# uingei/hevc

Hardware: AMD Instinct MI355X
Metric: encoded 1080p30 frames/sec/GPU; PSNR-Y parity vs libx265 at matched bitrate (higher is better)
Workload: dtype u8; 1 GPU; 1920x1080@30 SDR 8-bit Main, crf 19 capped by VBV maxrate 2940 kbps / bufsize 3528 kbit (the reference's libx265 operating point), 300-frame synthetic 'motion' clip per GPU, keyint 90 (4 closed GOPs of equal length), IPPP, full-search +-15, one clip per GPU, input resident in HBM

## Files before the change

### hevc_amd/csrc/kernels/common.h

```cpp
#pragma once
#include <stdint.h>

#if defined(__HIPCC__)
#include <hip/hip_runtime.h>
#define DEV __device__ __forceinline__
#define HD __host__ __device__
#define HDI __host__ __device__ inline
#define DEVCONST __device__ const
#define MIHEVC_GPU 1
#else
#define DEV inline
#define HD
#define HDI inline
#define DEVCONST static const
#define MIHEVC_GPU 0
#endif

#include "../../../include/mihevc.h"

namespace mihevc {

constexpr int CTU = 32;
constexpr int CTU_LOG2 = 5;
constexpr int PAD_Y = 80;
// ... 75 lines not shown
                         5, 5, 6, 6, 7, 8, 9, 10, 11, 13, 14, 16, 18, 20, 22, 24};
    for (int i = 0; i < 54; i++) t.tc[i] = (uint8_t)tcv[i];
    const int qs[6] = {26214, 23302, 20560, 18396, 16384, 14564}, ls[6] = {40, 45, 51, 57, 64, 72};
    for (int i = 0; i < 6; i++) { t.quant_scale[i] = (int16_t)qs[i]; t.level_scale[i] = (uint8_t)ls[i]; }
    const int cq[14] = {29, 30, 31, 32, 33, 33, 34, 34, 35, 35, 36, 36, 37, 37};
    for (int i = 0; i < 14; i++) t.chroma_qp[i] = (int8_t)cq[i];
    for (int ty = 0; ty < 4; ty++)
        for (int tx = 0; tx < 4; tx++) t.zorder[ty * 4 + tx] = (uint8_t)(((ty >> 1) * 2 + (tx >> 1)) * 4 + (ty & 1) * 2 + (tx & 1));
    return t;
}
DEVCONST Tables g_tab = make_tables();

DEV int iabs(int v) { return v < 0 ? -v : v; }
DEV int imin(int a, int b) { return a < b ? a : b; }
DEV int imax(int a, int b) { return a > b ? a : b; }
DEV int clip3(int lo, int hi, int v) { return v < lo ? lo : v > hi ? hi : v; }
DEV int ilog2u(unsigned v) { return 31 - __builtin_clz(v | 1); }
DEV int mvd_bits(int d)
{
    int a = iabs(d);
    return a == 0 ? 1 : a == 1 ? 3 : 3 + 2 * ilog2u((unsigned)a);
}
DEV int chroma_qp_of(int qp)
{
    int q = clip3(-12, 57, qp);
    return q < 30 ? q : q > 43 ? q - 6 : g_tab.chroma_qp[q - 30];
}
DEV int zaddr(int x, int y, int ctus_w)
{
    int bx = (x & 31) >> 2, by = (y & 31) >> 2, z = 0;
    for (int i = 0; i < 3; i++) z |= ((bx >> i) & 1) << (2 * i) | ((by >> i) & 1) << (2 * i + 1);
    return (((y >> CTU_LOG2) * ctus_w + (x >> CTU_LOG2)) << 6) | z;
}
DEV void node_geom(int node, int &x, int &y, int &log2n)
{
    if (node == 0) { x = 0; y = 0; log2n = 5; }
    else if (node < 5) { int q = node - 1; x = (q & 1) * 16; y = (q >> 1) * 16; log2n = 4; }
    else { int q = (node - 5) >> 2, s = (node - 5) & 3; x = (q & 1) * 16 + (s & 1) * 8; y = (q >> 1) * 16 + (s >> 1) * 8; log2n = 3; }
}
DEV int node_of_tile(int level, int tx, int ty)
{
    if (level == 0) return 0;
    int q = (ty >> 1) * 2 + (tx >> 1);
    return level == 1 ? 1 + q : 5 + q * 4 + (ty & 1) * 2 + (tx & 1);
}

DEV uint32_t sad_packed_u8(uint32_t a, uint32_t b, uint32_t acc)
{
#if MIHEVC_GPU
    return __builtin_amdgcn_sad_u8(a, b, acc);
#else
    for (int i = 0; i < 4; i++) acc += (uint32_t)iabs((int)((a >> (8 * i)) & 255) - (int)((b >> (8 * i)) & 255));
    return acc;
#endif
}
DEV uint32_t sad_packed_u16(uint32_t a, uint32_t b, uint32_t acc)
{
#if MIHEVC_GPU
    return __builtin_amdgcn_sad_u16(a, b, acc);
#else
    for (int i = 0; i < 2; i++) acc += (uint32_t)iabs((int)((a >> (16 * i)) & 65535) - (int)((b >> (16 * i)) & 65535));
    return acc;
#endif
}
DEV uint32_t load_u32(const void *p)
{
    uint32_t v;
    __builtin_memcpy(&v, p, 4);
    return v;
}
DEV uint32_t sad_row8(const uint8_t *a, const uint8_t *b, uint32_t acc)
{
    acc = sad_packed_u8(load_u32(a), load_u32(b), acc);
    return sad_packed_u8(load_u32(a + 4), load_u32(b + 4), acc);
}
DEV uint32_t sad_row8(const uint16_t *a, const uint16_t *b, uint32_t acc)
{
    for (int i = 0; i < 8; i += 2) acc = sad_packed_u16(load_u32(a + i), load_u32(b + i), acc);
    return acc;
}

DEV uint32_t pk_add16(uint32_t a, uint32_t b)
{
#if MIHEVC_GPU
    typedef short v2s __attribute__((ext_vector_type(2)));
    return __builtin_bit_cast(uint32_t, (v2s)(__builtin_bit_cast(v2s, a) + __builtin_bit_cast(v2s, b)));
#else
    return ((a + b) & 0xffffu) | (((a >> 16) + (b >> 16)) << 16);
#endif
}
DEV uint32_t pk_sub16(uint32_t a, uint32_t b)
{
#if MIHEVC_GPU
    typedef short v2s __attribute__((ext_vector_type(2)));
    return __builtin_bit_cast(uint32_t, (v2s)(__builtin_bit_cast(v2s, a) - __builtin_bit_cast(v2s, b)));
#else
    return ((a - b) & 0xffffu) | (((a >> 16) - (b >> 16)) << 16);
#endif
}
DEV uint32_t pk_max_i16(uint32_t a, uint32_t b)
{
#if MIHEVC_GPU
    uint32_t r;
    asm("v_pk_max_i16 %0, %1, %2" : "=v"(r) : "v"(a), "v"(b));
    return r;
#else
    const int al = (int16_t)(a & 0xffffu), ah = (int16_t)(a >> 16), bl = (int16_t)(b & 0xffffu), bh = (int16_t)(b >> 16);
    return (uint32_t)((al > bl ? al : bl) & 0xffff) | ((uint32_t)((ah > bh ? ah : bh) & 0xffff) << 16);
#endif
}

DEV uint32_t perm_bytes(uint32_t a, uint32_t b, uint32_t sel)
{
#if MIHEVC_GPU
    return __builtin_amdgcn_perm(a, b, sel);
#else
    const uint64_t ab = ((uint64_t)a << 32) | b;
    uint32_t r = 0;
    for (int i = 0; i < 4; i++) r |= (uint32_t)((ab >> (8 * ((sel >> (8 * i)) & 7))) & 255u) << (8 * i);
    return r;
#endif
}
DEV void transpose_bytes4(const uint32_t (&r)[4], uint32_t (&c)[4])
{
    const uint32_t t0 = perm_bytes(r[1], r[0], 0x05010400u), t1 = perm_bytes(r[1], r[0], 0x07030602u);
    const uint32_t t2 = perm_bytes(r[3], r[2], 0x05010400u), t3 = perm_bytes(r[3], r[2], 0x07030602u);
    c[0] = perm_bytes(t2, t0, 0x05040100u); c[1] = perm_bytes(t2, t0, 0x07060302u);
    c[2] = perm_bytes(t3, t1, 0x05040100u); c[3] = perm_bytes(t3, t1, 0x07060302u);
}

DEV bool wave_all(bool p)
{
#if MIHEVC_GPU
    return __all(p) != 0;
#else
    return p;
#endif
}

DEV uint64_t qsad_u8(uint64_t ref8, uint32_t cur, uint64_t acc)
{
#if MIHEVC_GPU
    return __builtin_amdgcn_qsad_pk_u16_u8(ref8, cur, acc);
#else
    uint64_t out = 0;
    for (int j = 0; j < 4; j++) {
        uint32_t w = (uint32_t)(ref8 >> (8 * j)), a = (uint32_t)((acc >> (16 * j)) & 0xffff);
        for (int i = 0; i < 4; i++) a += (uint32_t)iabs((int)((w >> (8 * i)) & 255) - (int)((cur >> (8 * i)) & 255));
        out |= (uint64_t)(a & 0xffff) << (16 * j);
    }
    return out;
#endif
}
DEV uint32_t align_bytes(uint32_t hi, uint32_t lo, int shift_bytes)
{
#if MIHEVC_GPU
    return __builtin_amdgcn_alignbyte(hi, lo, (uint32_t)shift_bytes);
#else
    return (uint32_t)(((((uint64_t)hi) << 32) | lo) >> (8 * shift_bytes));
#endif
}
template <typename T>
DEV void copy_window(T *lds, int ls, const T *plane, int pstride, int ox, int oy, int w, int h, int lo_x, int hi_x, int lo_y, int hi_y, int tid)
{
    constexpr int per = 4 / (int)sizeof(T);
    constexpr int CH = 6;
    const int dpr = w / per, col = tid & 31, rg = tid >> 5;
    for (int d = col; d < dpr; d += 32) {
        const int x = clip3(lo_x, hi_x - (per - 1), ox + d * per);
        for (int r0 = rg; r0 < h; r0 += CH * (NT / 32)) {
            uint32_t v[CH];
#pragma unroll
            for (int k = 0; k < CH; k++) {
                const int r = r0 + k * (NT / 32);
                if (r < h) v[k] = load_u32(plane + (ptrdiff_t)clip3(lo_y, hi_y, oy + r) * pstride + x);
            }
#pragma unroll
            for (int k = 0; k < CH; k++) {
                const int r = r0 + k * (NT / 32);
                if (r < h) __builtin_memcpy(__builtin_assume_aligned(lds + r * ls + d * per, 4), &v[k], 4);
            }
        }
    }
}

template <typename T>
DEV void load_ctu_source(T *dst, const Plane<const T> (&src)[3], int x0, int y0, int w, int h, int tid)
{
    constexpr int per = 4 / (int)sizeof(T);
    if (x0 + CTU <= w && y0 + CTU <= h) {
        constexpr int ND = 1536 / per, IT = (ND + NT - 1) / NT;
        uint32_t v[IT];
#pragma unroll
        for (int k = 0; k < IT; k++) {
            const int d = tid + k * NT;
            if (d < ND) {
                const int i = d * per, pl = i < 1024 ? 0 : 1 + ((i - 1024) >> 8), kk = pl ? (i - 1024) & 255 : i, x = pl ? kk & 15 : kk & 31, y = pl ? kk >> 4 : kk >> 5;
                v[k] = load_u32(src[pl].p + (size_t)((pl ? y0 >> 1 : y0) + y) * src[pl].stride + (pl ? x0 >> 1 : x0) + x);
            }
        }
#pragma unroll
        for (int k = 0; k < IT; k++) {
            const int d = tid + k * NT;
            if (d < ND) __builtin_memcpy(__builtin_assume_aligned(dst + d * per, 4), &v[k], 4);
        }
        return;
    }
    for (int i = tid; i < 1536; i += NT) {
        int pl, x, y;
        if (i < 1024) { pl = 0; x = i & 31; y = i >> 5; } else { int k = i - 1024; pl = 1 + (k >> 8); k &= 255; x = k & 15; y = k >> 4; }
        const int gx = (pl ? x0 >> 1 : x0) + x, gy = (pl ? y0 >> 1 : y0) + y, pw = pl ? w >> 1 : w, ph = pl ? h >> 1 : h;
        dst[i] = (gx < pw && gy < ph) ? src[pl].p[(size_t)gy * src[pl].stride + gx] : (T)0;
    }
}

DEV int wave_uniform(int v)
{
#if MIHEVC_GPU
    v = __builtin_amdgcn_readfirstlane(v);
#endif
    return v;
}
DEV int opaque_zero()
{
    int z = 0;
#if MIHEVC_GPU
    asm volatile("" : "+v"(z));
#endif
    return z;
}
DEV uint32_t load_u32_aligned(const void *p)
{
    uint32_t v;
    __builtin_memcpy(&v, __builtin_assume_aligned(p, 4), 4);
    return v;
}
DEV void store_u32_aligned(void *p, uint32_t v) { __builtin_memcpy(__builtin_assume_aligned(p, 4), &v, 4); }
DEV void store4(uint8_t *p, int v0, int v1, int v2, int v3) { store_u32_aligned(p, (uint32_t)v0 | (uint32_t)v1 << 8 | (uint32_t)v2 << 16 | (uint32_t)v3 << 24); }
DEV void store4(uint16_t *p, int v0, int v1, int v2, int v3)
{
    store_u32_aligned(p, (uint32_t)v0 | (uint32_t)v1 << 16);
    store_u32_aligned(p + 2, (uint32_t)v2 | (uint32_t)v3 << 16);
}
DEV void store4(int16_t *p, int v0, int v1, int v2, int v3)
{
    store_u32_aligned(p, ((uint32_t)v0 & 0xffffu) | (uint32_t)v1 << 16);
    store_u32_aligned(p + 2, ((uint32_t)v2 & 0xffffu) | (uint32_t)v3 << 16);
}
DEV void load_row15(const uint8_t *base, int idx, int (&px)[15])
{
    const int off = idx & 3;
    const uint8_t *p = base + (idx - off);
    uint32_t d[5];
#pragma unroll
    for (int k = 0; k < 5; k++) d[k] = load_u32_aligned(p + 4 * k);
    uint32_t r[4];
#pragma unroll
    for (int k = 0; k < 4; k++) r[k] = align_bytes(d[k + 1], d[k], off);
#pragma unroll
    for (int i = 0; i < 15; i++) px[i] = (int)((r[i >> 2] >> (8 * (i & 3))) & 255);
}
DEV void load_row15(const uint16_t *base, int idx, int (&px)[15])
{
    const int off = idx & 1;
    const uint16_t *p = base + (idx - off);
    uint32_t d[8];
#pragma unroll
    for (int k = 0; k < 8; k++) d[k] = load_u32_aligned(p + 2 * k);
    uint32_t r[8];
#pragma unroll
    for (int k = 0; k < 7; k++) r[k] = align_bytes(d[k + 1], d[k], 2 * off);
    r[7] = align_bytes(0, d[7], 2 * off);
#pragma unroll
    for (int i = 0; i < 15; i++) px[i] = (int)((r[i >> 1] >> (16 * (i & 1))) & 65535);
}

DEV void load_row8(const uint8_t *base, int idx, int (&px)[8])
{
    const int off = idx & 3;
    const uint8_t *p = base + (idx - off);
    const uint32_t d0 = load_u32_aligned(p), d1 = load_u32_aligned(p + 4), d2 = load_u32_aligned(p + 8);
    const uint32_t r0 = align_bytes(d1, d0, off), r1 = align_bytes(d2, d1, off);
#pragma unroll
    for (int i = 0; i < 4; i++) { px[i] = (int)((r0 >> (8 * i)) & 255); px[4 + i] = (int)((r1 >> (8 * i)) & 255); }
}
DEV void load_row8(const uint16_t *base, int idx, int (&px)[8])
{
    const int off = idx & 1;
    const uint16_t *p = base + (idx - off);
    uint32_t d[5];
#pragma unroll
    for (int k = 0; k < 5; k++) d[k] = load_u32_aligned(p + 2 * k);
#pragma unroll
    for (int k = 0; k < 4; k++) {
        const uint32_t r = align_bytes(d[k + 1], d[k], 2 * off);
        px[2 * k] = (int)(r & 65535); px[2 * k + 1] = (int)(r >> 16);
    }
}

DEV int dot4_i8(uint32_t a, uint32_t b, int acc)
{
#if MIHEVC_GPU
    return __builtin_amdgcn_sdot4((int)a, (int)b, acc, false);
#else
    for (int i = 0; i < 4; i++) acc += (int)(int8_t)(a >> (8 * i)) * (int)(int8_t)(b >> (8 * i));
    return acc;
#endif
}
DEV int dot2_i16(uint32_t a, uint32_t b, int acc)
{
#if MIHEVC_GPU
    typedef short v2s __attribute__((ext_vector_type(2)));
    v2s va, vb;
    __builtin_memcpy(&va, &a, 4);
    __builtin_memcpy(&vb, &b, 4);
    return __builtin_amdgcn_sdot2(va, vb, acc, false);
#else
    return acc + (int)(int16_t)(a & 0xffff) * (int)(int16_t)(b & 0xffff) + (int)(int16_t)(a >> 16) * (int)(int16_t)(b >> 16);
#endif
}

DEV uint32_t pack_lo16(int lo, int hi)
{
#if MIHEVC_GPU
    return __builtin_amdgcn_perm((uint32_t)hi, (uint32_t)lo, 0x05040100u);
#else
    return ((uint32_t)lo & 0xffffu) | ((uint32_t)hi << 16);
#endif
}

DEV int hadamard8_satd(int (&m)[8][8])
{
#pragma unroll
    for (int y = 0; y < 8; y++) {
#pragma unroll
        for (int st = 1; st < 8; st <<= 1)
#pragma unroll
            for (int i = 0; i < 8; i++)
                if (!(i & st)) { int p = m[y][i], q = m[y][i + st]; m[y][i] = p + q; m[y][i + st] = p - q; }
    }
    int s = 0;
#pragma unroll
    for (int x = 0; x < 8; x++) {
#pragma unroll
        for (int st = 1; st < 8; st <<= 1)
#pragma unroll
            for (int i = 0; i < 8; i++)
                if (!(i & st)) { int p = m[i][x], q = m[i + st][x]; m[i][x] = p + q; m[i + st][x] = p - q; }
#pragma unroll
        for (int i = 0; i < 8; i++) s += iabs(m[i][x]);
    }
    return (s + 2) >> 2;
}

DEV int hadamard8_ac(int (&m)[8][8])
{
#pragma unroll
    for (int y = 0; y < 8; y++) {
#pragma unroll
        for (int st = 1; st < 8; st <<= 1)
#pragma unroll
            for (int i = 0; i < 8; i++)
                if (!(i & st)) { int p = m[y][i], q = m[y][i + st]; m[y][i] = p + q; m[y][i + st] = p - q; }
    }
    int s = 0;
#pragma unroll
    for (int x = 0; x < 8; x++) {
#pragma unroll
        for (int st = 1; st < 8; st <<= 1)
#pragma unroll
            for (int i = 0; i < 8; i++)
                if (!(i & st)) { int p = m[i][x], q = m[i + st][x]; m[i][x] = p + q; m[i + st][x] = p - q; }
#pragma unroll
        for (int i = 0; i < 8; i++) if (x || i) s += iabs(m[i][x]);
    }
    return (s + 2) >> 2;
}

#if MIHEVC_GPU
#ifdef MIHEVC_PHASE_PROF
__device__ unsigned long long g_phase_prof[8 * 1024 * 3];
#endif
struct GpuExec {
    static DEV int lane_id()
    {
        int t = (int)threadIdx.x;
        asm volatile("" : "+v"(t));
        return t;
    }
// ... 88 lines not shown
```

### hevc_amd/csrc/kernels/inter.h

```cpp
#pragma once
#include "common.h"
#include "residual.h"

namespace mihevc {

template <typename T> struct InterArgs {
    Plane<const T> src[3];
    Plane<const T> ref[3];
    Plane<T> rec[3];
    int w, h, ctus_w;
    CostParams prm;
    const int16_t *centers;
    int32_t *me;
    mihevc_cu_rec *cu;
    int16_t *coef[3];
    unsigned long long *est;
    int sparse_coef;
    IpInfo *ip;
    Plane<const T> ref1[3];
    const int16_t *centers1;
    int32_t *me1;
};
template <typename T> DEV InterArgs<T> list1_view(const InterArgs<T> &a)
{
    InterArgs<T> b = a;
    for (int i = 0; i < 3; i++) b.ref[i] = a.ref1[i];
    b.centers = a.centers1; b.me = a.me1;
    return b;
}

DEVCONST int8_t kOff[9][2] = {{0, 0}, {-1, -1}, {0, -1}, {1, -1}, {-1, 0}, {1, 0}, {-1, 1}, {0, 1}, {1, 1}};
DEVCONST int8_t kRingSlot[8] = {4, 5, 2, 7, 1, 3, 6, 8};

template <typename T> struct PreArgs {
    Plane<const T> src, ref;
    uint8_t *lsrc, *lref;
    int w, h, bit_depth;
    int16_t *centers;
    unsigned *cost;
};
template <typename T> DEV void lowres_sample(const PreArgs<T> &a, int i)
{
    const int lw = a.w >> 2, n = lw * (a.h >> 2), sh = a.bit_depth - 8;
    if (i >= 2 * n) return;
    const Plane<const T> &p = i < n ? a.src : a.ref;
    const int k = i < n ? i : i - n, x = k % lw, y = k / lw;
    int s = 8 << sh;
#pragma unroll
    for (int j = 0; j < 4; j++) {
        const T *row = p.p + (ptrdiff_t)(4 * y + j) * p.stride + 4 * x;
        if (sizeof(T) == 1) {
            s = (int)sad_packed_u8(load_u32(row), 0u, (uint32_t)s);
        } else
            s += (int)row[0] + (int)row[1] + (int)row[2] + (int)row[3];
    }
    s >>= 4 + sh;
    (i < n ? a.lsrc : a.lref)[k] = (uint8_t)(s < 255 ? s : 255);
}
constexpr int PRE_SPAN = 2 * PRE_RANGE + 1;
constexpr int PRE_WIN_W = 40;
constexpr int PRE_WIN_STRIDE = 96;
struct PreShared {
    uint8_t blk[64];
    uint8_t win[(8 + 2 * PRE_RANGE) * PRE_WIN_STRIDE + 16];
    unsigned long long best;
    unsigned sad0;
};
template <typename T, class Ex> DEV void pre_search_program(Ex &ex, PreShared &s, const PreArgs<T> &a, int ctu)
{
    constexpr int R = PRE_RANGE, span = PRE_SPAN;
    const int lw = a.w >> 2, lh = a.h >> 2, wc = (lw + 7) >> 3, cx = ctu % wc, cy = ctu / wc;
    const int bw = lw - 8 * cx < 8 ? lw - 8 * cx : 8, bh = lh - 8 * cy < 8 ? lh - 8 * cy : 8;
    ex.phase([&](int tid) {
        if (tid < 64) { const int x = tid & 7, y = tid >> 3; s.blk[tid] = (x < bw && y < bh) ? a.lsrc[(8 * cy + y) * lw + 8 * cx + x] : (uint8_t)0; }
        if (8 * cx - R >= 0 && 8 * cx - R + PRE_WIN_W <= lw && 8 * cy - R >= 0 && 8 * cy + 8 + R <= lh) {
            constexpr int DPR = PRE_WIN_W / 4, ND = (8 + 2 * PRE_RANGE) * DPR, IT = (ND + NT - 1) / NT;
            uint32_t v[IT];
#pragma unroll
            for (int k = 0; k < IT; k++) {
                const int i = tid + k * NT;
                if (i < ND) v[k] = load_u32(a.lref + (size_t)(8 * cy - R + i / DPR) * lw + 8 * cx - R + 4 * (i % DPR));
            }
#pragma unroll
            for (int k = 0; k < IT; k++) {
                const int i = tid + k * NT;
                if (i < ND) store_u32_aligned(s.win + (i / DPR) * PRE_WIN_STRIDE + 4 * (i % DPR), v[k]);
            }
        } else {
            constexpr int NW = (8 + 2 * PRE_RANGE) * PRE_WIN_W, IT = (NW + NT - 1) / NT;
            uint8_t v[IT];
#pragma unroll
            for (int k = 0; k < IT; k++) {
                const int i = tid + k * NT;
                if (i < NW) v[k] = a.lref[clip3(0, lh - 1, 8 * cy + i / PRE_WIN_W - R) * lw + clip3(0, lw - 1, 8 * cx + i % PRE_WIN_W - R)];
            }
#pragma unroll
            for (int k = 0; k < IT; k++) {
                const int i = tid + k * NT;
                if (i < NW) s.win[(i / PRE_WIN_W) * PRE_WIN_STRIDE + i % PRE_WIN_W] = v[k];
            }
        }
        if (tid == 0) s.best = ~0ull;
    });
    ex.phase([&](int tid) {
        unsigned long long best = ~0ull;
        if (bw == 8 && bh == 8) {
            if (tid < 8 * span) {
                const int q = tid & 7, dyi = tid >> 3;
                uint64_t acc = 0;
#pragma unroll
                for (int y = 0; y < 8; y++) {
                    const uint8_t *w = s.win + (y + dyi) * PRE_WIN_STRIDE + 4 * q;
                    const uint32_t r0 = load_u32_aligned(w), r1 = load_u32_aligned(w + 4), r2 = load_u32_aligned(w + 8);
                    acc = qsad_u8(((uint64_t)r1 << 32) | r0, load_u32_aligned(s.blk + 8 * y), acc);
                    acc = qsad_u8(((uint64_t)r2 << 32) | r1, load_u32_aligned(s.blk + 8 * y + 4), acc);
                }
#pragma unroll
                for (int j = 0; j < 4; j++) {
                    const int dxi = 4 * q + j;
                    if (dxi >= span) continue;
                    const unsigned sad = (unsigned)((acc >> (16 * j)) & 0xffff);
                    if (dxi == R && dyi == R) s.sad0 = sad;
                    const unsigned long long key = ((unsigned long long)(4 * sad + (unsigned)(iabs(dxi - R) + iabs(dyi - R))) << 12) | (unsigned)(dyi * span + dxi);
                    best = key < best ? key : best;
                }
            }
        } else {
            for (int p = tid; p < span * span; p += NT) {
                const int dxi = p % span, dyi = p / span;
                unsigned sad = 0;
                for (int y = 0; y < bh; y++)
                    for (int x = 0; x < bw; x++) sad += (unsigned)iabs((int)s.blk[y * 8 + x] - (int)s.win[(y + dyi) * PRE_WIN_STRIDE + x + dxi]);
                if (dxi == R && dyi == R) s.sad0 = sad;
                const unsigned long long key = ((unsigned long long)(4 * sad + (unsigned)(iabs(dxi - R) + iabs(dyi - R))) << 12) | (unsigned)p;
                best = key < best ? key : best;
            }
        }
        if (best != ~0ull) ex.atomic_min(&s.best, best);
    });
    ex.phase([&](int tid) {
        if (tid != 0) return;
        int p = (int)(s.best & 4095);
        const unsigned sad_best = (unsigned)(((s.best >> 12) - (unsigned)(iabs(p % span - R) + iabs(p / span - R))) >> 2);
        if (2 * sad_best >= s.sad0) p = R * span + R;
        a.centers[2 * ctu] = (int16_t)(4 * (p % span - R));
        a.centers[2 * ctu + 1] = (int16_t)(4 * (p / span - R));
        if (a.cost) a.cost[ctu] = sad_best;
    });
}

DEV bool mv_rows_ok(int y, int n, int my, int h, int top, int bottom)
{
    const int ly0 = y + (my >> 2) - ((my & 3) ? 3 : 0), ly1 = y + n - 1 + (my >> 2) + ((my & 3) ? 4 : 0);
    const int cy0 = (y >> 1) + (my >> 3) - ((my & 7) ? 1 : 0), cy1 = (y >> 1) + (n >> 1) - 1 + (my >> 3) + ((my & 7) ? 2 : 0);
    if (top && (ly0 < 0 || cy0 < 0)) return false;
    if (bottom && (ly1 > h - 1 || cy1 > (h >> 1) - 1)) return false;
    return true;
}
DEV int clamp_center_y(int sy, int y0, int R, int h, int top, int bottom)
{
    const int ctu_h = h - y0 < CTU ? h - y0 : CTU;
    if (bottom && sy > h - (y0 + ctu_h) - R) sy = h - (y0 + ctu_h) - R;
    if (top && sy < R - y0) sy = R - y0;
    return sy;
}

template <typename T> struct MeShared {
    uint8_t src[32 * 32];
    unsigned long long best[21];
    uint8_t valid[21];
    unsigned nodeok[2 * MAX_RANGE + 1];
};
HDI int me_spanx(int R) { return ((2 * R + 1) + 3) & ~3; }
HDI int me_win_w(int R) { return 32 + me_spanx(R); }
HDI int me_win_stride(int R)
{
    int u = (me_win_w(R) + 4 + 3) >> 2;
    while ((u & 15) != 8) u++;
    return u << 2;
}
HDI int me_win_elems(int R) { return (32 + 2 * R) * me_win_stride(R) + 16; }

DEV void quad_block_row(const uint8_t *src, const uint8_t *ref, int ws, unsigned (&out)[4][4])
{
    uint64_t acc[4] = {0, 0, 0, 0};
#pragma unroll 2
    for (int r = 0; r < 8; r++) {
        uint32_t rr[9], cc[8];
#pragma unroll
        for (int d = 0; d < 9; d++) rr[d] = load_u32_aligned(ref + r * ws + 4 * d);
#pragma unroll
        for (int d = 0; d < 8; d++) cc[d] = load_u32_aligned(src + r * 32 + 4 * d);
#pragma unroll
        for (int d = 0; d < 8; d++) acc[d >> 1] = qsad_u8(((uint64_t)rr[d + 1] << 32) | rr[d], cc[d], acc[d >> 1]);
    }
#pragma unroll
    for (int b = 0; b < 4; b++)
#pragma unroll
        for (int j = 0; j < 4; j++) out[b][j] = (unsigned)((acc[b] >> (16 * j)) & 0xffff);
}
DEV void copy_window_msb(uint8_t *lds, int ls, const uint16_t *plane, int pstride, int ox, int oy, int w, int h, int lo_x, int hi_x, int lo_y, int hi_y, int sh, int tid)
{
    const int dpr = w / 4, col = tid & 31, rg = tid >> 5;
    for (int r = rg; r < h; r += NT / 32) {
        const int y = clip3(lo_y, hi_y, oy + r);
        const uint16_t *srow = plane + (ptrdiff_t)y * pstride;
        for (int d = col; d < dpr; d += 32) {
            const int x = clip3(lo_x, hi_x - 3, ox + d * 4);
            const uint32_t a = load_u32(srow + x), b = load_u32(srow + x + 2);
            const uint32_t v = ((a & 0xffffu) >> sh) | (((a >> 16) >> sh) << 8) | (((b & 0xffffu) >> sh) << 16) | (((b >> 16) >> sh) << 24);
            store_u32_aligned(lds + r * ls + d * 4, v);
        }
    }
}
DEV void copy_window_msb(uint8_t *lds, int ls, const uint8_t *plane, int pstride, int ox, int oy, int w, int h, int lo_x, int hi_x, int lo_y, int hi_y, int, int tid)
{
    copy_window<uint8_t>(lds, ls, plane, pstride, ox, oy, w, h, lo_x, hi_x, lo_y, hi_y, tid);
}

template <typename T, class Ex>
DEV void me_search_program(Ex &ex, MeShared<T> &s, uint8_t *win, const InterArgs<T> &a, int ctu)
{
    const int msb = sizeof(T) == 1 ? 0 : a.prm.bit_depth - 8;

    const int R = a.prm.me_range, spany = 2 * R + 1, spanx = me_spanx(R), quads = spanx >> 2, ws = me_win_stride(R), ww = me_win_w(R), wh = 32 + 2 * R;
    const int x0 = (ctu % a.ctus_w) * CTU, y0 = (ctu / a.ctus_w) * CTU;
    const int mct = a.prm.mc_top, mcb = a.prm.mc_bottom;
    const int sx = a.centers ? a.centers[2 * ctu] : 0, sy0 = a.centers ? a.centers[2 * ctu + 1] : 0;
    const int sy = (mct || mcb) ? clamp_center_y(sy0, y0, R, a.h, mct, mcb) : sy0;
    ex.phase([&](int tid) {
        if (sizeof(T) == 1 && x0 + CTU <= a.w && y0 + CTU <= a.h) {
            const uint32_t v = load_u32(a.src[0].p + (size_t)(y0 + (tid >> 3)) * a.src[0].stride + x0 + 4 * (tid & 7));
            store_u32_aligned(s.src + 4 * tid, v);
        } else
        for (int i = tid; i < 1024; i += NT) {
            int x = x0 + (i & 31), y = y0 + (i >> 5);
            s.src[i] = (x < a.w && y < a.h) ? (uint8_t)(a.src[0].p[(size_t)y * a.src[0].stride + x] >> msb) : (uint8_t)0;
        }
        copy_window_msb(win, ws, a.ref[0].p, a.ref[0].stride, x0 + sx - R, y0 + sy - R, ww, wh, -PAD_Y, a.w + PAD_Y - 1, -PAD_Y, a.h + PAD_Y - 1, msb, tid);
        if (tid < 21) {
            int nx, ny, nl;
            node_geom(tid, nx, ny, nl);
            s.valid[tid] = x0 + nx + (1 << nl) <= a.w && y0 + ny + (1 << nl) <= a.h;
            s.best[tid] = ~0ull;
        }
        for (int dyi = tid; dyi < spany; dyi += NT) {
            unsigned bits = 0;
            for (int n = 0; n < 21; n++) {
                int nx, ny, nl;
                node_geom(n, nx, ny, nl);
                const bool in_pic = x0 + nx + (1 << nl) <= a.w && y0 + ny + (1 << nl) <= a.h;
                if (in_pic && (!(mct || mcb) || mv_rows_ok(y0 + ny, 1 << nl, 4 * (sy + dyi - R), a.h, mct, mcb))) bits |= 1u << n;
            }
            s.nodeok[dyi] = bits;
        }
    });
    ex.phase([&](int tid) {
#ifdef MIHEVC_EXP_DPP_MIN
        for (int it0 = 0; it0 < quads * spany; it0 += NT) {
            const int item = it0 + tid < quads * spany ? it0 + tid : 0;
            const int q = item % quads, dyi = item / quads;
            const unsigned ok = it0 + tid < quads * spany ? s.nodeok[dyi] : 0u, pos0 = (unsigned)(dyi * spanx + 4 * q);
#else
        for (int item = tid; item < quads * spany; item += NT) {
            const int q = item % quads, dyi = item / quads;
            const unsigned ok = s.nodeok[dyi], pos0 = (unsigned)(dyi * spanx + 4 * q);
#endif
            const int by = mvd_bits(4 * (dyi - R)), ksh = 6 + msb;
            const uint8_t *srcp = s.src + opaque_zero();
            unsigned bitsj[4], s32[4] = {0, 0, 0, 0};
#pragma unroll
            for (int j = 0; j < 4; j++) bitsj[j] = ((unsigned)(a.prm.lambda_sad_q4 * (mvd_bits(4 * (4 * q + j - R)) + by)) << 2) | (unsigned)j;
            auto consider = [&](int node, const unsigned (&sad)[4]) {
                unsigned k = (sad[0] << ksh) + bitsj[0];
#pragma unroll
                for (int j = 1; j < 4; j++) { const unsigned kj = (sad[j] << ksh) + bitsj[j]; k = kj < k ? kj : k; }
#ifdef MIHEVC_EXP_DPP_MIN
                unsigned long long key = ((ok >> node) & 1) ? (((unsigned long long)(k >> 2) << 16) | (pos0 + (k & 3))) : ~0ull;
                auto step = [&](auto ctrl, auto row_mask) {
                    const unsigned lo = (unsigned)key, hi = (unsigned)(key >> 32);
                    const unsigned tl = (unsigned)__builtin_amdgcn_update_dpp((int)lo, (int)lo, decltype(ctrl)::value, decltype(row_mask)::value, 0xf, false);
                    const unsigned th = (unsigned)__builtin_amdgcn_update_dpp((int)hi, (int)hi, decltype(ctrl)::value, decltype(row_mask)::value, 0xf, false);
                    const unsigned long long t = ((unsigned long long)th << 32) | tl;
                    key = t < key ? t : key;
                };
                step(std::integral_constant<int, 0x111>{}, std::integral_constant<int, 0xf>{});
                step(std::integral_constant<int, 0x112>{}, std::integral_constant<int, 0xf>{});
                step(std::integral_constant<int, 0x114>{}, std::integral_constant<int, 0xf>{});
                step(std::integral_constant<int, 0x118>{}, std::integral_constant<int, 0xf>{});
                step(std::integral_constant<int, 0x142>{}, std::integral_constant<int, 0xa>{});
                step(std::integral_constant<int, 0x143>{}, std::integral_constant<int, 0xc>{});
                if ((tid & 63) == 63 && key < ex.peek(&s.best[node])) ex.atomic_min(&s.best[node], key);
#else
                if (!((ok >> node) & 1)) return;
                const unsigned long long key = ((unsigned long long)(k >> 2) << 16) | (pos0 + (k & 3));
                if (key < ex.peek(&s.best[node])) ex.atomic_min(&s.best[node], key);
#endif
            };
#pragma unroll
            for (int half = 0; half < 2; half++) {
                unsigned s16[2][4] = {{0, 0, 0, 0}, {0, 0, 0, 0}};
#pragma unroll
                for (int r2 = 0; r2 < 2; r2++) {
                    const int br = half * 2 + r2;
                    unsigned o[4][4];
                    quad_block_row(srcp + br * 8 * 32, win + (br * 8 + dyi) * ws + 4 * q, ws, o);
#pragma unroll
                    for (int b = 0; b < 4; b++) {
#pragma unroll
                        for (int j = 0; j < 4; j++) s16[b >> 1][j] += o[b][j];
                        consider(5 + (half * 2 + (b >> 1)) * 4 + r2 * 2 + (b & 1), o[b]);
                    }
                }
#pragma unroll
                for (int h2 = 0; h2 < 2; h2++) {
#pragma unroll
                    for (int j = 0; j < 4; j++) s32[j] += s16[h2][j];
                    consider(1 + half * 2 + h2, s16[h2]);
                }
            }
            consider(0, s32);
        }
    });
    ex.phase([&](int tid) {
        if (tid < 21) {
            int32_t *o = a.me + ((size_t)ctu * 21 + tid) * 3;
            if (s.valid[tid]) {
                int p = (int)(s.best[tid] & 0xffff);
                o[0] = 4 * (sx + p % spanx - R); o[1] = 4 * (sy + p / spanx - R); o[2] = (int32_t)(s.best[tid] >> 16);
            } else { o[0] = 0; o[1] = 0; o[2] = -1; }
        }
    });
}

template <typename T> struct InterShared {
    ResidualShared rs;
    T src[1536];
    T pred[1536];
    int mvx[21], mvy[21];
    unsigned cost[21];
    uint8_t valid[21];
    int satd[3][1][16];
    unsigned nsum[21];
    unsigned fsum[8][21];
    unsigned long long rbest[21];
    unsigned j16[4];
    int use16[4], use32;
    uint8_t alias[3][16];
    int tile_mvx[16], tile_mvy[16];
    uint8_t tile_node[16];
    uint8_t chosen[21];
    unsigned est;
    unsigned ip_cost, ip_act, ip_tiles;
    unsigned long long ip_sse;
    unsigned tu_dc[3][16], tu_dz[3][16], tu_bits[3][16], tu_zero[3];
};
constexpr int FRAC_PAIR_SUM = 8 * NT;
constexpr int FRAC_SCRATCH = FRAC_PAIR_SUM + NT;
static_assert(FRAC_SCRATCH <= (int)(sizeof(ResidualShared::scratch) / 4), "the fractional search's exchange must fit rs.scratch");
HDI int mc_win_y(int R) { return (32 + 2 * (R + 3) + 8 + 3) & ~3; }
HDI int mc_win_y_stride(int R) { return mc_win_y(R) + 4; }
HDI int mc_win_c(int R) { return (16 + (R + 3) + 8 + 3) & ~3; }
HDI int mc_win_c_stride(int R) { return mc_win_c(R) + 4; }

struct InterLds { size_t y, u, v, bytes; };
template <typename T> HDI constexpr size_t inter_win_in() { return offsetof(InterShared<T>, rs) + offsetof(ResidualShared, scratch) + 4 * (size_t)FRAC_SCRATCH; }
template <typename T> HDI constexpr size_t inter_win_out() { return (sizeof(InterShared<T>) + 15) & ~(size_t)15; }
template <typename T> HDI InterLds inter_lds(int R)
{
    const size_t n[3] = {((size_t)mc_win_y(R) * mc_win_y_stride(R) + 16) * sizeof(T), ((size_t)mc_win_c(R) * mc_win_c_stride(R) + 16) * sizeof(T),
                         ((size_t)mc_win_c(R) * mc_win_c_stride(R) + 16) * sizeof(T)};
    const size_t hi = offsetof(InterShared<T>, rs) + offsetof(ResidualShared, scratch) + sizeof(ResidualShared::scratch);
    size_t in = inter_win_in<T>(), out = inter_win_out<T>(), at[3];
    for (int i = 0; i < 3; i++) {
        const size_t r = (n[i] + 15) & ~(size_t)15;
        if (in + r <= hi) { at[i] = in; in += r; } else { at[i] = out; out += r; }
    }
    return InterLds{at[0], at[1], at[2], out};
}

template <typename T>
DEV int luma_tile(const T *win, int i00, int ws, int fx, int fy, int bit_depth, const T *diff_src, int src_stride, T *pred_out, int pred_stride)
{
    const int8_t *tx = g_tab.luma_tap[fx], *ty = g_tab.luma_tap[fy];
    const int shift1 = bit_depth - 8, shift3 = 14 - bit_depth, maxv = (1 << bit_depth) - 1;
    int acc[8][8];
#pragma unroll
    for (int j = 0; j < 8; j++)
#pragma unroll
        for (int i = 0; i < 8; i++) acc[j][i] = 0;
    for (int r = 0; r < 15; r++) {
        int px[15];
        load_row15(win, i00 + (r - 3) * ws - 3, px);
        int hv[8];
#pragma unroll
        for (int i = 0; i < 8; i++) {
            int v = 0;
#pragma unroll
            for (int k = 0; k < 8; k++) v += tx[k] * px[i + k];
            hv[i] = v >> shift1;
        }
#pragma unroll
        for (int j = 0; j < 8; j++) {
            int k = r - j;
            if (k >= 0 && k < 8) {
                int t = ty[k];
#pragma unroll
                for (int i = 0; i < 8; i++) acc[j][i] += t * hv[i];
            }
        }
    }
    const int off = 1 << (shift3 - 1);
#pragma unroll
    for (int j = 0; j < 8; j++)
#pragma unroll
        for (int i = 0; i < 8; i++) {
            int v = clip3(0, maxv, ((acc[j][i] >> 6) + off) >> shift3);
            if (diff_src) acc[j][i] = (int)diff_src[j * src_stride + i] - v;
            else pred_out[j * pred_stride + i] = (T)v;
        }
    return diff_src ? hadamard8_satd(acc) : 0;
}

DEV int luma_tile(const uint8_t *win, int i00, int ws, int fx, int fy, int bit_depth, const uint8_t *diff_src, int src_stride, uint8_t *pred_out,
                  int pred_stride)
{
    const uint32_t tlo = load_u32(&g_tab.luma_tap[fx][0]), thi = load_u32(&g_tab.luma_tap[fx][4]);
    uint32_t typ[4];
#pragma unroll
    for (int m = 0; m < 4; m++) typ[m] = pack_lo16(g_tab.luma_tap[fy][2 * m], g_tab.luma_tap[fy][2 * m + 1]);
    int acc[8][8], prev[8];
#pragma unroll
    for (int j = 0; j < 8; j++)
#pragma unroll
        for (int i = 0; i < 8; i++) acc[j][i] = 0;
#pragma unroll
    for (int r = 0; r < 15; r++) {
        const int idx = i00 + (r - 3) * ws - 3, off = idx & 3;
        const uint8_t *p = win + (idx - off);
        uint32_t d[5], a[12];
#pragma unroll
        for (int k = 0; k < 5; k++) d[k] = load_u32_aligned(p + 4 * k);
        uint32_t q[4];
#pragma unroll
        for (int k = 0; k < 4; k++) q[k] = align_bytes(d[k + 1], d[k], off) ^ 0x80808080u;
#pragma unroll
        for (int k = 0; k < 3; k++) {
            a[4 * k] = q[k];
            a[4 * k + 1] = align_bytes(q[k + 1], q[k], 1);
            a[4 * k + 2] = align_bytes(q[k + 1], q[k], 2);
            a[4 * k + 3] = align_bytes(q[k + 1], q[k], 3);
        }
        int hv[8];
#pragma unroll
        for (int i = 0; i < 8; i++) hv[i] = dot4_i8(a[i], tlo, dot4_i8(a[i + 4], thi, 128 * 64));
        if (r > 0) {
#pragma unroll
            for (int i = 0; i < 8; i++) {
                const uint32_t pr = pack_lo16(prev[i], hv[i]);
#pragma unroll
                for (int m = 0; m < 4; m++) {
                    const int j = r - 1 - 2 * m;
                    if (j >= 0 && j < 8) acc[j][i] = dot2_i16(pr, typ[m], acc[j][i]);
                }
            }
        }
#pragma unroll
        for (int i = 0; i < 8; i++) prev[i] = hv[i];
    }
    (void)bit_depth;
#pragma unroll
    for (int j = 0; j < 8; j++)
#pragma unroll
        for (int i = 0; i < 8; i++) {
            int v = clip3(0, 255, ((acc[j][i] >> 6) + 32) >> 6);
// ... 804 lines not shown
```

Measured before the change: 5776 frames/s.

## Restructure ME SAD search with duplicated window, packed sums and filtered atomic updates

The integer motion-search window is stored twice in LDS at an offset, so each qsad can read an aligned 64-bit pair with one ds_read_b64 instead of assembling it from two 32-bit loads. SADs stay packed as 16-bit lanes and are combined with pk_add16 and v_mad_u32_u16 into cost keys. A per-node relaxed filter value skips most atomic_min calls on the shared best key. Interior CTUs skip the per-row node-validity mask through a compile-time specialisation, and the stride-96 case gets a constant stride with more unrolling. The price is twice the LDS for the window, which may reduce occupancy, and the filter reads and writes are racy but only act as a hint before the atomic.

```diff
diff --git a/hevc_amd/csrc/kernels/common.h b/hevc_amd/csrc/kernels/common.h
--- a/hevc_amd/csrc/kernels/common.h
+++ b/hevc_amd/csrc/kernels/common.h
@@ -251,6 +251,27 @@
     return out;
 #endif
 }
+template <int HI> DEV uint32_t mad_u16_half(uint32_t packed, uint32_t mul, uint32_t add)
+{
+#if MIHEVC_GPU
+    uint32_t r;
+    if (HI) asm("v_mad_u32_u16 %0, %1, %2, %3 op_sel:[1,0,0,0]" : "=v"(r) : "v"(packed), "s"(mul), "v"(add));
+    else asm("v_mad_u32_u16 %0, %1, %2, %3" : "=v"(r) : "v"(packed), "s"(mul), "v"(add));
+    return r;
+#else
+    return ((packed >> (16 * HI)) & 0xffffu) * (mul & 0xffffu) + add;
+#endif
+}
+DEV uint64_t lds_read_u64(const uint8_t *p)
+{
+#if MIHEVC_GPU
+    return *(const volatile __attribute__((address_space(3))) uint64_t *)p;
+#else
+    uint64_t v;
+    __builtin_memcpy(&v, p, 8);
+    return v;
+#endif
+}
 DEV uint32_t align_bytes(uint32_t hi, uint32_t lo, int shift_bytes)
 {
 #if MIHEVC_GPU
@@ -260,7 +281,7 @@
 #endif
 }
 template <typename T>
-DEV void copy_window(T *lds, int ls, const T *plane, int pstride, int ox, int oy, int w, int h, int lo_x, int hi_x, int lo_y, int hi_y, int tid)
+DEV void copy_window(T *lds, int ls, const T *plane, int pstride, int ox, int oy, int w, int h, int lo_x, int hi_x, int lo_y, int hi_y, int tid, int dup = 0)
 {
     constexpr int per = 4 / (int)sizeof(T);
     constexpr int CH = 6;
@@ -277,7 +298,10 @@
 #pragma unroll
             for (int k = 0; k < CH; k++) {
                 const int r = r0 + k * (NT / 32);
-                if (r < h) __builtin_memcpy(__builtin_assume_aligned(lds + r * ls + d * per, 4), &v[k], 4);
+                if (r < h) {
+                    __builtin_memcpy(__builtin_assume_aligned(lds + r * ls + d * per, 4), &v[k], 4);
+                    if (dup) __builtin_memcpy(__builtin_assume_aligned(lds + dup + r * ls + d * per, 4), &v[k], 4);
+                }
             }
         }
     }
@@ -334,6 +358,8 @@
     __builtin_memcpy(&v, __builtin_assume_aligned(p, 4), 4);
     return v;
 }
+DEV unsigned relaxed_load(const unsigned *p) { return __atomic_load_n(p, __ATOMIC_RELAXED); }
+DEV void relaxed_store(unsigned *p, unsigned v) { __atomic_store_n(p, v, __ATOMIC_RELAXED); }
 DEV void store_u32_aligned(void *p, uint32_t v) { __builtin_memcpy(__builtin_assume_aligned(p, 4), &v, 4); }
 DEV void store4(uint8_t *p, int v0, int v1, int v2, int v3) { store_u32_aligned(p, (uint32_t)v0 | (uint32_t)v1 << 8 | (uint32_t)v2 << 16 | (uint32_t)v3 << 24); }
 DEV void store4(uint16_t *p, int v0, int v1, int v2, int v3)
diff --git a/hevc_amd/csrc/kernels/inter.h b/hevc_amd/csrc/kernels/inter.h
--- a/hevc_amd/csrc/kernels/inter.h
+++ b/hevc_amd/csrc/kernels/inter.h
@@ -1,6 +1,8 @@
 #pragma once
 #include "common.h"
 #include "residual.h"
+
+#include <type_traits>
 
 namespace mihevc {
 
@@ -168,6 +170,7 @@
 template <typename T> struct MeShared {
     uint8_t src[32 * 32];
     unsigned long long best[21];
+    unsigned filt[21];
     uint8_t valid[21];
     unsigned nodeok[2 * MAX_RANGE + 1];
 };
@@ -179,27 +182,31 @@
     while ((u & 15) != 8) u++;
     return u << 2;
 }
-HDI int me_win_elems(int R) { return (32 + 2 * R) * me_win_stride(R) + 16; }
-
-DEV void quad_block_row(const uint8_t *src, const uint8_t *ref, int ws, unsigned (&out)[4][4])
-{
-    uint64_t acc[4] = {0, 0, 0, 0};
-#pragma unroll 2
+HDI int me_win_one(int R) { return (32 + 2 * R) * me_win_stride(R) + 16; }
+HDI int me_win_dup(int R)
+{
+    int d = (me_win_one(R) + 3) & ~3;
+    while ((d & 255) != 124) d += 4;
+    return d;
+}
+HDI int me_win_elems(int R) { return me_win_dup(R) + me_win_one(R); }
+
+template <int UNROLL> DEV void quad_block_row(const uint8_t *src, const uint8_t *pe, const uint8_t *po, int ws, uint64_t (&acc)[4])
+{
+    acc[0] = acc[1] = acc[2] = acc[3] = 0;
+#pragma unroll UNROLL
     for (int r = 0; r < 8; r++) {
-        uint32_t rr[9], cc[8];
-#pragma unroll
-        for (int d = 0; d < 9; d++) rr[d] = load_u32_aligned(ref + r * ws + 4 * d);
+        uint64_t rr[8];
+        uint32_t cc[8];
+#pragma unroll
+        for (int d = 0; d < 8; d += 2) { rr[d] = lds_read_u64(pe + r * ws + 4 * d); rr[d + 1] = lds_read_u64(po + r * ws + 4 * d); }
 #pragma unroll
         for (int d = 0; d < 8; d++) cc[d] = load_u32_aligned(src + r * 32 + 4 * d);
 #pragma unroll
-        for (int d = 0; d < 8; d++) acc[d >> 1] = qsad_u8(((uint64_t)rr[d + 1] << 32) | rr[d], cc[d], acc[d >> 1]);
-    }
-#pragma unroll
-    for (int b = 0; b < 4; b++)
-#pragma unroll
-        for (int j = 0; j < 4; j++) out[b][j] = (unsigned)((acc[b] >> (16 * j)) & 0xffff);
-}
-DEV void copy_window_msb(uint8_t *lds, int ls, const uint16_t *plane, int pstride, int ox, int oy, int w, int h, int lo_x, int hi_x, int lo_y, int hi_y, int sh, int tid)
+        for (int d = 0; d < 8; d++) acc[d >> 1] = qsad_u8(rr[d], cc[d], acc[d >> 1]);
+    }
+}
+DEV void copy_window_msb(uint8_t *lds, int ls, const uint16_t *plane, int pstride, int ox, int oy, int w, int h, int lo_x, int hi_x, int lo_y, int hi_y, int sh, int tid, int dup)
 {
     const int dpr = w / 4, col = tid & 31, rg = tid >> 5;
     for (int r = rg; r < h; r += NT / 32) {
@@ -210,12 +217,13 @@
             const uint32_t a = load_u32(srow + x), b = load_u32(srow + x + 2);
             const uint32_t v = ((a & 0xffffu) >> sh) | (((a >> 16) >> sh) << 8) | (((b & 0xffffu) >> sh) << 16) | (((b >> 16) >> sh) << 24);
             store_u32_aligned(lds + r * ls + d * 4, v);
-        }
-    }
-}
-DEV void copy_window_msb(uint8_t *lds, int ls, const uint8_t *plane, int pstride, int ox, int oy, int w, int h, int lo_x, int hi_x, int lo_y, int hi_y, int, int tid)
-{
-    copy_window<uint8_t>(lds, ls, plane, pstride, ox, oy, w, h, lo_x, hi_x, lo_y, hi_y, tid);
+            store_u32_aligned(lds + dup + r * ls + d * 4, v);
+        }
+    }
+}
+DEV void copy_window_msb(uint8_t *lds, int ls, const uint8_t *plane, int pstride, int ox, int oy, int w, int h, int lo_x, int hi_x, int lo_y, int hi_y, int, int tid, int dup)
+{
+    copy_window<uint8_t>(lds, ls, plane, pstride, ox, oy, w, h, lo_x, hi_x, lo_y, hi_y, tid, dup);
 }
 
 template <typename T, class Ex>
@@ -223,11 +231,12 @@
 {
     const int msb = sizeof(T) == 1 ? 0 : a.prm.bit_depth - 8;
 
-    const int R = a.prm.me_range, spany = 2 * R + 1, spanx = me_spanx(R), quads = spanx >> 2, ws = me_win_stride(R), ww = me_win_w(R), wh = 32 + 2 * R;
+    const int R = a.prm.me_range, spany = 2 * R + 1, spanx = me_spanx(R), quads = spanx >> 2, ws = me_win_stride(R), ww = me_win_w(R), wh = 32 + 2 * R, dup = me_win_dup(R);
     const int x0 = (ctu % a.ctus_w) * CTU, y0 = (ctu / a.ctus_w) * CTU;
     const int mct = a.prm.mc_top, mcb = a.prm.mc_bottom;
     const int sx = a.centers ? a.centers[2 * ctu] : 0, sy0 = a.centers ? a.centers[2 * ctu + 1] : 0;
     const int sy = (mct || mcb) ? clamp_center_y(sy0, y0, R, a.h, mct, mcb) : sy0;
+    const bool all_ok = x0 + CTU <= a.w && y0 + CTU <= a.h && !(mct || mcb);
     ex.phase([&](int tid) {
         if (sizeof(T) == 1 && x0 + CTU <= a.w && y0 + CTU <= a.h) {
             const uint32_t v = load_u32(a.src[0].p + (size_t)(y0 + (tid >> 3)) * a.src[0].stride + x0 + 4 * (tid & 7));
@@ -237,90 +246,90 @@
             int x = x0 + (i & 31), y = y0 + (i >> 5);
             s.src[i] = (x < a.w && y < a.h) ? (uint8_t)(a.src[0].p[(size_t)y * a.src[0].stride + x] >> msb) : (uint8_t)0;
         }
-        copy_window_msb(win, ws, a.ref[0].p, a.ref[0].stride, x0 + sx - R, y0 + sy - R, ww, wh, -PAD_Y, a.w + PAD_Y - 1, -PAD_Y, a.h + PAD_Y - 1, msb, tid);
+        copy_window_msb(win, ws, a.ref[0].p, a.ref[0].stride, x0 + sx - R, y0 + sy - R, ww, wh, -PAD_Y, a.w + PAD_Y - 1, -PAD_Y, a.h + PAD_Y - 1, msb, tid, dup);
         if (tid < 21) {
             int nx, ny, nl;
             node_geom(tid, nx, ny, nl);
             s.valid[tid] = x0 + nx + (1 << nl) <= a.w && y0 + ny + (1 << nl) <= a.h;
             s.best[tid] = ~0ull;
-        }
-        for (int dyi = tid; dyi < spany; dyi += NT) {
-            unsigned bits = 0;
-            for (int n = 0; n < 21; n++) {
-                int nx, ny, nl;
-                node_geom(n, nx, ny, nl);
-                const bool in_pic = x0 + nx + (1 << nl) <= a.w && y0 + ny + (1 << nl) <= a.h;
-                if (in_pic && (!(mct || mcb) || mv_rows_ok(y0 + ny, 1 << nl, 4 * (sy + dyi - R), a.h, mct, mcb))) bits |= 1u << n;
-            }
-            s.nodeok[dyi] = bits;
-        }
-    });
-    ex.phase([&](int tid) {
-#ifdef MIHEVC_EXP_DPP_MIN
-        for (int it0 = 0; it0 < quads * spany; it0 += NT) {
-            const int item = it0 + tid < quads * spany ? it0 + tid : 0;
-            const int q = item % quads, dyi = item / quads;
-            const unsigned ok = it0 + tid < quads * spany ? s.nodeok[dyi] : 0u, pos0 = (unsigned)(dyi * spanx + 4 * q);
-#else
+            s.filt[tid] = ~0u;
+        }
+        if (!all_ok && tid < spany) s.nodeok[tid] = 0;
+    });
+    if (!all_ok) ex.phase([&](int tid) {
+        for (int p = tid; p < spany * 21; p += NT) {
+            const int dyi = p / 21, n = p - dyi * 21;
+            int nx, ny, nl;
+            node_geom(n, nx, ny, nl);
+            const bool in_pic = x0 + nx + (1 << nl) <= a.w && y0 + ny + (1 << nl) <= a.h;
+            if (in_pic && (!(mct || mcb) || mv_rows_ok(y0 + ny, 1 << nl, 4 * (sy + dyi - R), a.h, mct, mcb))) ex.atomic_or(&s.nodeok[dyi], 1u << n);
+        }
+    });
+    auto search = [&](int tid, auto all, auto stride) {
+        constexpr bool ALL = decltype(all)::value;
+        constexpr int WS = decltype(stride)::value;
+        const int ws = WS ? WS : me_win_stride(R);
+        const int ksh = 6 + msb;
+        const unsigned kmul = 1u << ksh;
         for (int item = tid; item < quads * spany; item += NT) {
             const int q = item % quads, dyi = item / quads;
-            const unsigned ok = s.nodeok[dyi], pos0 = (unsigned)(dyi * spanx + 4 * q);
-#endif
-            const int by = mvd_bits(4 * (dyi - R)), ksh = 6 + msb;
+            const unsigned ok = ALL ? ~0u : s.nodeok[dyi], pos0 = (unsigned)(dyi * spanx + 4 * q);
+            const int by = mvd_bits(4 * (dyi - R));
             const uint8_t *srcp = s.src + opaque_zero();
+            const uint8_t *wl = win + dyi * ws + 4 * q, *pe = wl + ((q & 1) ? dup : 0), *po = wl + 4 + ((q & 1) ? 0 : dup);
             unsigned bitsj[4], s32[4] = {0, 0, 0, 0};
 #pragma unroll
             for (int j = 0; j < 4; j++) bitsj[j] = ((unsigned)(a.prm.lambda_sad_q4 * (mvd_bits(4 * (4 * q + j - R)) + by)) << 2) | (unsigned)j;
-            auto consider = [&](int node, const unsigned (&sad)[4]) {
-                unsigned k = (sad[0] << ksh) + bitsj[0];
-#pragma unroll
-                for (int j = 1; j < 4; j++) { const unsigned kj = (sad[j] << ksh) + bitsj[j]; k = kj < k ? kj : k; }
-#ifdef MIHEVC_EXP_DPP_MIN
-                unsigned long long key = ((ok >> node) & 1) ? (((unsigned long long)(k >> 2) << 16) | (pos0 + (k & 3))) : ~0ull;
-                auto step = [&](auto ctrl, auto row_mask) {
-                    const unsigned lo = (unsigned)key, hi = (unsigned)(key >> 32);
-                    const unsigned tl = (unsigned)__builtin_amdgcn_update_dpp((int)lo, (int)lo, decltype(ctrl)::value, decltype(row_mask)::value, 0xf, false);
-                    const unsigned th = (unsigned)__builtin_amdgcn_update_dpp((int)hi, (int)hi, decltype(ctrl)::value, decltype(row_mask)::value, 0xf, false);
-                    const unsigned long long t = ((unsigned long long)th << 32) | tl;
-                    key = t < key ? t : key;
-                };
-                step(std::integral_constant<int, 0x111>{}, std::integral_constant<int, 0xf>{});
-                step(std::integral_constant<int, 0x112>{}, std::integral_constant<int, 0xf>{});
-                step(std::integral_constant<int, 0x114>{}, std::integral_constant<int, 0xf>{});
-                step(std::integral_constant<int, 0x118>{}, std::integral_constant<int, 0xf>{});
-                step(std::integral_constant<int, 0x142>{}, std::integral_constant<int, 0xa>{});
-                step(std::integral_constant<int, 0x143>{}, std::integral_constant<int, 0xc>{});
-                if ((tid & 63) == 63 && key < ex.peek(&s.best[node])) ex.atomic_min(&s.best[node], key);
-#else
-                if (!((ok >> node) & 1)) return;
-                const unsigned long long key = ((unsigned long long)(k >> 2) << 16) | (pos0 + (k & 3));
-                if (key < ex.peek(&s.best[node])) ex.atomic_min(&s.best[node], key);
-#endif
+            auto submit = [&](int node, unsigned k) {
+                if (k <= relaxed_load(&s.filt[node])) {
+                    relaxed_store(&s.filt[node], k | 3u);
+                    ex.atomic_min(&s.best[node], ((unsigned long long)(k >> 2) << 16) | (pos0 + (k & 3)));
+                }
             };
+            auto consider = [&](int node, uint64_t sad4) {
+                if (!ALL && !((ok >> node) & 1)) return;
+                const uint32_t lo = (uint32_t)sad4, hi = (uint32_t)(sad4 >> 32);
+                const unsigned k0 = mad_u16_half<0>(lo, kmul, bitsj[0]), k1 = mad_u16_half<1>(lo, kmul, bitsj[1]);
+                const unsigned k2 = mad_u16_half<0>(hi, kmul, bitsj[2]), k3 = mad_u16_half<1>(hi, kmul, bitsj[3]);
+                const unsigned k01 = k1 < k0 ? k1 : k0, k23 = k3 < k2 ? k3 : k2;
+                submit(node, k23 < k01 ? k23 : k01);
+            };
 #pragma unroll
             for (int half = 0; half < 2; half++) {
-                unsigned s16[2][4] = {{0, 0, 0, 0}, {0, 0, 0, 0}};
+                uint64_t s16[2] = {0, 0};
 #pragma unroll
                 for (int r2 = 0; r2 < 2; r2++) {
                     const int br = half * 2 + r2;
-                    unsigned o[4][4];
-                    quad_block_row(srcp + br * 8 * 32, win + (br * 8 + dyi) * ws + 4 * q, ws, o);
+                    uint64_t o[4];
+                    quad_block_row<(WS ? 4 : 2)>(srcp + br * 8 * 32, pe + br * 8 * ws, po + br * 8 * ws, ws, o);
 #pragma unroll
                     for (int b = 0; b < 4; b++) {
-#pragma unroll
-                        for (int j = 0; j < 4; j++) s16[b >> 1][j] += o[b][j];
+                        s16[b >> 1] = (uint64_t)pk_add16((uint32_t)s16[b >> 1], (uint32_t)o[b]) | ((uint64_t)pk_add16((uint32_t)(s16[b >> 1] >> 32), (uint32_t)(o[b] >> 32)) << 32);
                         consider(5 + (half * 2 + (b >> 1)) * 4 + r2 * 2 + (b & 1), o[b]);
                     }
                 }
 #pragma unroll
                 for (int h2 = 0; h2 < 2; h2++) {
-#pragma unroll
-                    for (int j = 0; j < 4; j++) s32[j] += s16[h2][j];
+                    const uint32_t lo = (uint32_t)s16[h2], hi = (uint32_t)(s16[h2] >> 32);
+                    s32[0] = mad_u16_half<0>(lo, 1u, s32[0]); s32[1] = mad_u16_half<1>(lo, 1u, s32[1]);
+                    s32[2] = mad_u16_half<0>(hi, 1u, s32[2]); s32[3] = mad_u16_half<1>(hi, 1u, s32[3]);
                     consider(1 + half * 2 + h2, s16[h2]);
                 }
             }
-            consider(0, s32);
-        }
+            if (ALL || (ok & 1)) {
+                unsigned k = (s32[0] << ksh) + bitsj[0];
+#pragma unroll
+                for (int j = 1; j < 4; j++) { const unsigned kj = (s32[j] << ksh) + bitsj[j]; k = kj < k ? kj : k; }
+                submit(0, k);
+            }
+        }
+    };
+    ex.phase([&](int tid) {
+        if (ws == 96) {
+            if (all_ok) search(tid, std::true_type{}, std::integral_constant<int, 96>{});
+            else search(tid, std::false_type{}, std::integral_constant<int, 96>{});
+        } else if (all_ok) search(tid, std::true_type{}, std::integral_constant<int, 0>{});
+        else search(tid, std::false_type{}, std::integral_constant<int, 0>{});
     });
     ex.phase([&](int tid) {
         if (tid < 21) {
```

Measured after the change: 5557 frames/s. 0.962x the previous value.
